# XiangLi2022/CM-TTS

Hardware: AMD Instinct MI355X
Metric: mel-frames/s (text->mel hot path, consistency sampling T=4) (higher is better)
Workload: dtype f32

## Files before the change

### cm-tts_amd/csrc/cmtts_api.hip

```cpp
#include <hip/hip_runtime.h>
#include <limits.h>
#include <math.h>
#include <stdio.h>
#include <stdlib.h>
#include <string.h>

#include <algorithm>
#include <map>
#include <string>
#include <vector>

#include "../../include/cmtts_hip.h"
#include "internal_hooks.h"
#include "conv_args.h"
#include "kernels.h"
#include "resblock_args.h"
#include "persist_args.h"
#include "cond_gemm.h"
#include "resblock_pair.h"
#include "inproj.h"
#include "attention.h"
#include "text_state.h"
#include "stream_windows.h"

// ... 385 lines not shown
int launch(const ConvArgs& a, int epi, int nbatch, hipStream_t s) {
    const int r = cmtts_launch_conv(&a, epi, nbatch, (void*)s);
    if (r != 0) return fail(r, "conv launch failed (unsupported shape or HIP launch error)");
    return 0;
}

struct Carver {
    char* base;
    size_t off = 0;
    explicit Carver(void* b) : base((char*)b) {}
    template <class T>
    T* take(size_t n) {
        off = (off + 255) & ~(size_t)255;
        T* p = (T*)(base + off);
        off += n * sizeof(T);
        return p;
    }
};

struct Profile {
    bool on = false;
    std::vector<hipEvent_t> ev;
    size_t used = 0;
    int stride = 1;
    long seen = 0;
} g_prof;

bool g_fused_resblock = true;
int g_persist_tail = 1;
extern "C" int cmtts_launch_conv_xresq(const ConvArgs* a, const float* wq, int nbatch, void* stream, int form);
int g_ffn_wino = 1;
int g_ffn_fused = 1;
int g_inproj_fused = 1;
int g_step_cache = 1;
int g_persist_wino = 3;
int g_voc_wino = 1;
int g_voc_wino64_k = 7;
int g_voc_wino43 = 1;
int g_voc_qpair = 1;
int g_voc_wino64 = 1;
int g_voc_pair3 = 1;
int g_voc_pairw = 1;
int g_voc_pair128 = 1;
int g_voc_rb16 = 1;
int g_voc_upsT = 1;
int g_voc_xl16 = 1;
int g_pred_xl = 1;
int g_pred_head = 1;
int g_text_xres = 7;
int g_attn_fused = 1;
int g_voc_xl = 1;
int g_voc_pair = 1;
int g_qkv_nt = 0;
int g_stats_mlp = 1;
int g_cwt_in_phoneme = 1;
int g_xres_small = 1;
int g_ffn_xres = 1;
int g_split_resblock = 1;
int g_cond_gemm16 = 1;
int g_cond_gemm = 1;
int g_persist = 1;
unsigned* g_tmo_host = nullptr;
int check_device_flag(bool before_launch = false) {
    if (!g_tmo_host) return 0;
    unsigned v = __atomic_load_n(g_tmo_host, __ATOMIC_RELAXED);
    if (!v) return 0;
// ... 784 lines not shown
int g_cond_inkernel = 1;
inline bool C_IS_256(const cmtts_config& c) { return c.res_channels == 256; }
bool CondFactors::usable(const cmtts_model* m) const {
    return g_cond_factored && p1 && mel2ph && p_idx && m->precision == 0 && m->cond_p2 && g_fused_resblock;
}
int cond_factored(cmtts_model* m, const DenWs& w, const CondFactors& f, int B, int T, hipStream_t s) {
    const cmtts_config& c = m->cfg;
    const int r = cmtts_launch_cond_expand(f.p1, f.ldp, f.L, m->cond_p2, c.pitch_bins, f.mel2ph, f.p_idx, w.cp, B, c.res_layers * c.res_channels, T, (void*)s);
    return r == 0 ? 0 : fail(CMTTS_E_HIP, "cond_expand launch failed");
}
int cond_phoneme_factor(cmtts_model* m, const float* out1, int B, int Lp, float* p1, hipStream_t s) {
    const cmtts_config& c = m->cfg;
    if (!m->cond_p2) return fail(CMTTS_E_UNSUPPORTED, "factored conditioner projections are not available for this model");
    CondGemmArgs g;
    memset(&g, 0, sizeof(g));
    g.X = out1; g.Wf = m->cond_all_f; g.bias = m->cond_zero_bias; g.Y = p1;
    g.B = B; g.T = Lp; g.M = c.res_layers * c.res_channels; g.K = c.hidden; g.force = 1;
    g.flat = 1;
    const long tiles = ((long)B * Lp + 63) / 64;
    const int npass = g.M / 512;
    int best = 1;
    double best_t = 1e30;
    for (int sp = 1; sp <= npass; ++sp) {
        const int ppg = (npass + sp - 1) / sp, groups = (npass + ppg - 1) / ppg;
        const long wg = tiles * groups, cap = persist_blocks();
        const double t = (double)((wg + cap - 1) / cap) * ppg;
        if (t < best_t - 1e-9) { best_t = t; best = sp; }
    }
    g.row_split = best;
    const int r = cmtts_launch_cond_gemm(&g, (void*)s);
    return r == 0 ? 0 : fail(r == -2 ? CMTTS_E_UNSUPPORTED : CMTTS_E_HIP, "cond_gemm (phoneme factor) launch failed");
}

int step_embedding(cmtts_model* m, const DenWs& w, const float* timesteps, const float* spk, int B, hipStream_t s,
                   float t_host = NAN) {
    const cmtts_config& c = m->cfg;
    const int C = c.res_channels, NL = c.res_layers;
    if (c.multi_speaker && !spk) return fail(CMTTS_E_INVALID, "speaker_emb is required for a multi-speaker model");
    const bool cacheable = g_step_cache && t_host == t_host;
    if (cacheable) {
        for (const cmtts_model::StepRow& e : m->step_rows)
            if (e.t == t_host && hipEventQuery(e.ready) == hipSuccess) {
                k_broadcast_row(e.row, w.dproj, B, NL * C, s);
                if (c.multi_speaker) {
                    k_dense_small(spk, c.hidden, 1, m->sproj_wt, nullptr, nullptr, w.sproj, B, c.hidden, NL * C, DENSE_NONE, s);
                    k_add_rows(w.dproj, w.sproj, w.dp, (long)B * NL * C, s);
                }
                return 0;
            }
    }
    k_diff_embed(timesteps, m->omega_res, w.emb, B, C, s);
    k_dense_small(w.emb, C, 1, m->mlp0_wt, nullptr, nullptr, w.e1, B, C, 4 * C, DENSE_MISH, s);
    k_dense_small(w.e1, 4 * C, 1, m->mlp2_wt, nullptr, nullptr, w.e2, B, 4 * C, C, DENSE_NONE, s);
    k_dense_small(w.e2, C, 1, m->dproj_wt, nullptr, nullptr, w.dproj, B, C, NL * C, DENSE_NONE, s);
    if (c.multi_speaker) {
        k_dense_small(spk, c.hidden, 1, m->sproj_wt, nullptr, nullptr, w.sproj, B, c.hidden, NL * C, DENSE_NONE, s);
        k_dense_small(w.e2, C, 1, m->dproj_wt, nullptr, w.sproj, w.dp, B, C, NL * C, DENSE_NONE, s);
    }
    if (cacheable && m->step_rows.size() < 16) {
        bool known = false;
        for (const cmtts_model::StepRow& e : m->step_rows) known = known || e.t == t_host;
        if (!known) {
            cmtts_model::StepRow e{t_host, nullptr, nullptr};
            void* p = nullptr;
            if (hipMalloc(&p, (size_t)NL * C * sizeof(float)) == hipSuccess && hipEventCreateWithFlags(&e.ready, hipEventDisableTiming) == hipSuccess) {
                e.row = (float*)p;
// ... 24 lines not shown
    *halo_zeroed = false;
    int rin = -2;
    if (g_inproj_fused && m->in_proj_f) {
        InProjArgs ia;
        memset(&ia, 0, sizeof(ia));
        ia.x = x_src; ia.scale = in_scale; ia.wf = m->in_proj_f; ia.bias = m->in_proj.bias; ia.h = w.h;
        ia.B = B; ia.T = T; ia.M = M; ia.C = C;
        const bool persist_path = g_fused_resblock && g_persist && NL <= PERSIST_MAX_LAYERS;
        if (persist_path) { ia.zero = w.halo; ia.zero_f4 = (long)(cmtts_persist_halo_bytes(B, T) / 16); }
        rin = cmtts_launch_inproj(&ia, (void*)s);
        if (rin == -3) return fail(CMTTS_E_HIP, "inproj launch failed");
        *halo_zeroed = rin == 0 && persist_path && cmtts_persist_halo_bytes(B, T) % 16 == 0;
    }
    if (rin != 0) {
        k_mel_prep(x_src, nullptr, in_scale, w.hin, B, T, M, s);
        ConvArgs a = conv_args(m->in_proj, w.hin, T, T, (long)M * T, w.h, T, cs, T);
        a.out[0].act = ACT_RELU;
        CHK(launch(a, EPI_PLAIN, B, s));
    }
    if (embed) CHK(step_embedding(m, w, timesteps, spk, B, s, t_host));
    return 0;
}

int batch_invariant_form(const cmtts_model* m) {
    if (!m->batch_invariant || m->precision != 0 || !m->winograd || !g_persist_wino || !m->res[0].w3w) return 0;
    return m->winograd == 1 && g_persist_wino == 3 && m->res[0].w3w43 ? 1 : -1;
}
int check_batch_invariant(const cmtts_model* m) {
    if (batch_invariant_form(m) >= 0) return 0;
    return fail(CMTTS_E_UNSUPPORTED, "batch_invariant: the persistent denoiser stack runs the F(2,3) form (model option \"winograd\" = 2), "
                                     "which has no per-layer counterpart; set \"winograd\" to 1 or 0");
}

int denoiser_core(cmtts_model* m, const DenWs& w, const float* x_src, float in_scale, const float* timesteps,
                  const float* cond_ct, const float* spk, int B, int T, const MelPost& post, hipStream_t s, bool embed = true,
                  SideStream* pending = nullptr, float t_host = NAN,
                  const CondFactors* cfk = nullptr, bool* cp_ready = nullptr) {
    CHK(check_device_flag(true));
    const cmtts_config& c = m->cfg;
    const int C = c.res_channels, NL = c.res_layers, M = c.n_mels;
    const long cs = (long)C * T;
    bool halo_zeroed = false;
    CHK(denoiser_prologue(m, w, x_src, in_scale, timesteps, spk, B, T, s, embed, t_host, &halo_zeroed));
    if (pending) CHK(branch_join(pending));
    const float* dp = m->cfg.multi_speaker ? w.dp : w.dproj;
    const bool unfused = !g_fused_resblock;
    float* hcur = w.h;
    float* halt = w.u;
    bool layers_done = false;
    if (!unfused && g_persist && NL <= PERSIST_MAX_LAYERS) {
        PersistArgs pa;
        memset(&pa, 0, sizeof(pa));
        pa.x0 = w.h; pa.cp = w.cp; pa.cp_bstride = (long)NL * C * T;
        pa.dp = dp; pa.d = w.dproj; pa.vec_stride = (long)NL * C;
        pa.skip = w.skip; pa.halo = w.halo; pa.tmo = g_tmo_host;
        pa.B = B; pa.T = T; pa.NL = NL;
        pa.halo_zeroed = halo_zeroed;
        const int prec = m->precision;
        if (cfk && !(cp_ready && *cp_ready)) {
            pa.fact = 1; pa.p1 = cfk->p1; pa.p2 = m->cond_p2; pa.mel2ph = (const long long*)cfk->mel2ph; pa.pidx = (const long long*)cfk->p_idx;
            pa.ldp = cfk->ldp; pa.Lph = cfk->L; pa.ld2 = c.pitch_bins;
            pa.p1t = cfk->p1t; pa.p2t = m->cond_p2t;
        }
        if (g_persist_tail && m->skip_f && m->outp_f) {
            pa.tail = 1;
            pa.Wsf = m->skip_f; pa.bs = m->skip_proj.bias; pa.Wpf = m->outp_f; pa.bp = m->out_proj.bias;
            pa.skip_div = (float)sqrt((double)NL); pa.n_mels = M;
            pa.xold = post.xold; pa.noise = post.noise; pa.c_out = post.c_out; pa.c_skip = post.c_skip; pa.nstd = post.nstd;
            pa.out = post.out;
        }
        pa.wino = g_persist_wino && m->winograd && !prec && m->res[0].w3w && w.pst;
        if (pa.wino && g_persist_wino == 3 && m->winograd == 1 && m->res[0].w3w43) pa.wino = 3;
        pa.xst = w.pst;
        for (int l = 0; l < NL; ++l) {
            pa.W3f[l] = prec ? (const float*)m->res[l].w3f16[prec - 1] : (pa.wino == 3 ? m->res[l].w3w43 : pa.wino ? m->res[l].w3w : m->res[l].w3f);
            pa.Wof[l] = prec ? (const float*)m->res[l].wof16[prec - 1] : m->res[l].wof;
            pa.b3[l] = m->res[l].b3f; pa.bo[l] = m->res[l].outp.bias;
        }
        const bool prof = g_prof.on && g_prof.used + 2 <= g_prof.ev.size();
        const int need = cmtts_persist_plan(B, T, NL, persist_blocks(), g_persist == 2);
        if (need) CHK(persist_admit(s, need, persist_blocks()));
        if (prof) (void)hipEventRecord(g_prof.ev[g_prof.used], s);
        const int rc = prec ? cmtts_launch_denoiser_persist_lp(&pa, prec, persist_blocks(), g_persist == 2, (void*)s)
                            : cmtts_launch_denoiser_persist(&pa, persist_blocks(), g_persist == 2, (void*)s);
        if (rc == -3) return fail(CMTTS_E_HIP, "persistent denoiser launch failed");
        if (rc == 0) {
            CHK(persist_launched(s, need));
            if (prof) { (void)hipEventRecord(g_prof.ev[g_prof.used + 1], s); g_prof.used += 2; }
            layers_done = true;
            if (pa.tail) return 0;
        }
    }
    if (!layers_done && cfk && !(cp_ready && *cp_ready)) {
        CHK(cond_factored(m, w, *cfk, B, T, s));
        if (cp_ready) *cp_ready = true;
    }
    const bool w43 = batch_invariant_form(m) > 0;
    for (int l = 0; l < NL && !layers_done; ++l) {
        const ResLayer& R = m->res[l];
        const bool prof = g_prof.on && g_prof.used + 2 <= g_prof.ev.size() && (g_prof.seen++ % g_prof.stride) == 0;
        if (!unfused) {
            ResArgs ra;
            memset(&ra, 0, sizeof(ra));
            ra.x_in = hcur; ra.cp = w.cp + (long)l * C * T; ra.cp_bstride = (long)NL * C * T;
            ra.dp = dp + (long)l * C; ra.d = w.dproj + (long)l * C;
            ra.x_out = halt; ra.skip = w.skip;
            ra.W3f = R.w3f; ra.b3 = R.b3f; ra.Wof = R.wof; ra.bo = R.outp.bias;
            ra.vec_stride = (long)NL * C; ra.B = B; ra.T = T; ra.accum_skip = l > 0; ra.flag = g_tmo_host;
            if (prof) (void)hipEventRecord(g_prof.ev[g_prof.used], s);
            int lrc;
            if (m->precision == 0 || m->precision == 3) {
                const long tiles32 = (long)((T + 31) / 32) * B;
                ra.z = w.zb;
                if (w43) {
                    ra.W3f = R.w3w43;
                    lrc = cmtts_launch_resblock_w43(&ra, (void*)s);
                } else if (g_split_resblock == 2 || (g_split_resblock == 1 && tiles32 <= SPLIT_MAX_TILES)) lrc = cmtts_launch_resblock_split(&ra, (void*)s);
                else lrc = cmtts_launch_resblock(&ra, (void*)s);
// ... 547 lines not shown
    if (g_fused_resblock) CHK(cond_projections(m, w, cond_ct, B, T, ss ? ss->side : s));
    const MelPost post = {nullptr, nullptr, 1.0f, 0.0f, 0.0f, out};
    CHK(denoiser_core(m, w, x, 1.0f, timesteps, cond_ct, speaker_emb, B, T, post, s, true, ss));
    HIPCHK(hipGetLastError());
    return 0;
}

int cmtts_schedule(const cmtts_model* m, int n_steps, float* sigmas, float* renoise_std) {
    if (!m || !sigmas || !renoise_std || n_steps < 1) return fail(CMTTS_E_INVALID, "cmtts_schedule: bad argument");
    const cmtts_config& c = m->cfg;
    if (n_steps == 1) {
        sigmas[0] = c.sigma_max;
        renoise_std[0] = -1.0f;
        return 0;
    }
    const double rho = c.rho, tmax = pow((double)c.sigma_max, 1.0 / rho), tmin = pow((double)c.sigma_min, 1.0 / rho);
    for (int i = 0; i < n_steps; ++i) {
        const double tsi = 0.0, tsn = (i + 1 == n_steps) ? 1.0 : 0.0;
        const double t = pow(tmax + tsi / 1.0 * (tmin - tmax), rho);
        double nt = pow(tmax + tsn / 1.0 * (tmin - tmax), rho);
        nt = nt < c.sigma_min ? (double)c.sigma_min : (nt > c.sigma_max ? (double)c.sigma_max : nt);
        sigmas[i] = (float)t;
        renoise_std[i] = (float)sqrt(nt * nt - (double)c.sigma_min * (double)c.sigma_min);
    }
    return 0;
}

}
namespace {
int sample_core(cmtts_model* m, const DenWs& w, const float* noise, long noise_stride, const float* cond_ct, const float* speaker_emb, int B,
                int T, int n_steps, const float* sigmas, const float* renoise_std, float* mel, hipStream_t s, const CondFactors* cf = nullptr) {
    const cmtts_config& c = m->cfg;
    const long nel = (long)B * T * c.n_mels;
    SideStream* ss = g_fused_resblock ? side_for(s) : nullptr;
    if (ss) CHK(branch_fork(ss));
    const CondFactors* cfk = nullptr;
    CondFactors cf_local;
    bool cp_ready = false;
    if (g_fused_resblock) {
        if (cf && cf->usable(m)) {
            const bool inkernel = g_cond_inkernel && g_persist && g_persist_tail && m->skip_f && m->outp_f && c.res_layers <= PERSIST_MAX_LAYERS &&
                                  cmtts_persist_plan(B, T, c.res_layers, persist_blocks(), g_persist == 2) > 0;
            if (inkernel && cf->ldp <= T && m->cond_p2t && C_IS_256(c)) {
                cf_local = *cf;
                if (!cf_local.p1t) {
                    k_transpose(cf->p1, w.cp, B * c.res_layers, c.res_channels, cf->ldp, ss ? ss->side : s);
                    cf_local.p1t = w.cp;
                }
                cfk = &cf_local;
            } else CHK(cond_factored(m, w, *cf, B, T, ss ? ss->side : s));
        } else CHK(cond_projections(m, w, cond_ct, B, T, ss ? ss->side : s));
    }
    k_scale(noise, w.xcur, nel, c.sigma_max, s);
    const float smin = c.sigma_min, sd2 = c.sigma_data * c.sigma_data;
    for (int i = 0; i < n_steps; ++i) {
        const float sg = sigmas[i];
        const float dm = sg - smin;
        const float c_skip = sd2 / (dm * dm + sd2);
        const float rt = sqrtf(sg * sg + sd2);
        const float c_out = dm * c.sigma_data / rt;
        const float c_in = 1.0f / rt;
        const float t_resc = 250.0f * logf(sg + 1e-44f);
        const bool new_sigma = i == 0 || sigmas[i] != sigmas[i - 1];
        const bool embed_side = i == 0 && ss != nullptr;
        if (new_sigma) k_fill_float(w.tbuf, t_resc, B, embed_side ? ss->side : s);
        if (embed_side) CHK(step_embedding(m, w, w.tbuf, speaker_emb, B, ss->side, t_resc));
        const bool last = i + 1 == n_steps;
        const bool renoise = renoise_std[i] >= 0.0f;
        const MelPost post = {w.xcur, renoise ? noise + (long)(1 + i) * noise_stride : nullptr, c_out, c_skip,
                              renoise ? renoise_std[i] : 0.0f, last ? mel : w.xcur};
        CHK(denoiser_core(m, w, w.xcur, c_in, w.tbuf, cond_ct, speaker_emb, B, T, post, s, new_sigma && !embed_side, i == 0 ? ss : nullptr, t_resc, cfk, &cp_ready));
    }
    HIPCHK(hipGetLastError());
    return 0;
}

DenWs den_slice(const cmtts_config& c, const DenWs& w, int b0, int T) {
    const long C = c.res_channels, NL = c.res_layers, M = c.n_mels;
    DenWs v = w;
    v.hin += (long)b0 * M * T; v.h += b0 * C * T; v.u += b0 * C * T; v.zb += b0 * C * T; v.skip += b0 * C * T;
    v.emb += b0 * C; v.e1 += b0 * 4 * C; v.e2 += b0 * C; v.dproj += b0 * NL * C; v.sproj += b0 * NL * C; v.dp += b0 * NL * C;
    v.tbuf += b0; v.xcur += (long)b0 * T * M; v.cp += (long)b0 * NL * C * T;
    return v;
}
}
extern "C" {

int cmtts_sample(cmtts_model* m, const float* noise, const float* cond_ct, const float* speaker_emb, int B, int T,
                 int n_steps, const float* sigmas, const float* renoise_std, float* mel, void* ws, size_t ws_bytes,
                 void* stream) {
    if (!m || !m->finalized) return fail(CMTTS_E_INVALID, "model not finalized");
    if (!noise || !cond_ct || !mel || !ws || !sigmas || !renoise_std || B <= 0 || T <= 0 || n_steps < 1)
        return fail(CMTTS_E_INVALID, "cmtts_sample: bad argument");
    CHK(check_batch_invariant(m));
    const cmtts_config& c = m->cfg;
    DenWs w = carve_den(c, B, T, ws);
    if (ws_bytes < w.bytes) return fail(CMTTS_E_WORKSPACE, "denoiser workspace too small");
    return sample_core(m, w, noise, (long)B * T * c.n_mels, cond_ct, speaker_emb, B, T, n_steps, sigmas, renoise_std, mel, (hipStream_t)stream);
}

int cmtts_sample_factored(cmtts_model* m, const float* noise, const float* cond_ct, const float* speaker_emb, int B, int T,
                          int n_steps, const float* sigmas, const float* renoise_std, float* mel, void* ws, size_t ws_bytes,
                          void* stream, const float* cond_p1, int p1_ld, int L, const int64_t* mel2ph, const int64_t* p_idx) {
    return cmtts_sample_factored_t(m, noise, cond_ct, speaker_emb, B, T, n_steps, sigmas, renoise_std, mel, ws, ws_bytes, stream, cond_p1, nullptr, p1_ld, L,
// ... 687 lines not shown
    bool found;
    const int prev = knob_set(tab, sizeof(tab) / sizeof(tab[0]), name, value, &found);
    if (found) return prev;
    return fail(CMTTS_E_INVALID, "cmtts_model_set_option: unknown option");
}

int cmtts_vocoder_set_option(cmtts_vocoder* v, const char* name, int value) {
    if (!v || !name) return fail(CMTTS_E_INVALID, "cmtts_vocoder_set_option: null argument");
    const Knob tab[] = {
        {"ups16", &v->ups16, 0, 1},
        {"winograd", &v->winograd, 0, 1},
        {"batch_invariant", &v->batch_invariant, 0, 1},
    };
    bool found;
    const int prev = knob_set(tab, sizeof(tab) / sizeof(tab[0]), name, value, &found);
    if (found) return prev;
    return fail(CMTTS_E_INVALID, "cmtts_vocoder_set_option: unknown option");
}

int cmtts_internal_set(const char* name, int value) {
    if (!name) return fail(CMTTS_E_INVALID, "cmtts_internal_set: null name");
    static const Knob tab[] = {
        {"qkv_nt", &g_qkv_nt, 0, 3},
        {"cwt_in_phoneme", &g_cwt_in_phoneme, 0, 1},
        {"pred_xres", &g_pred_xres, 0, 1},
        {"xres_small", &g_xres_small, 0, 1},
        {"cond_inkernel", &g_cond_inkernel, 0, 1},
        {"cond_factored", &g_cond_factored, 0, 1},
        {"cond_gemm16", &g_cond_gemm16, 0, 1},
        {"cond_gemm", &g_cond_gemm, 0, 2},
        {"persist_tail", &g_persist_tail, 0, 1},
        {"persist_wino", &g_persist_wino, 0, 3},
        {"inproj_fused", &g_inproj_fused, 0, 1},
        {"ffn_xres", &g_ffn_xres, 0, 1},
        {"ffn_wino", &g_ffn_wino, 0, 2},
        {"ffn_fused", &g_ffn_fused, 0, 1},
        {"text_xres", &g_text_xres, 0, 15},
        {"attn_fused", &g_attn_fused, 0, 1},
        {"pred_xl", &g_pred_xl, 0, 1},
        {"pred_head", &g_pred_head, 0, 1},
        {"voc_pair", &g_voc_pair, 0, 2},
        {"voc_pair3", &g_voc_pair3, 0, 1},
        {"voc_pairw", &g_voc_pairw, 0, 1},
        {"voc_pair128", &g_voc_pair128, 0, 1},
        {"voc_rb16", &g_voc_rb16, 0, 2},
        {"voc_xl", &g_voc_xl, 0, 1},
        {"voc_wino64_k", &g_voc_wino64_k, 3, 99},
        {"voc_wino43", &g_voc_wino43, 0, 3},
        {"voc_qpair", &g_voc_qpair, 0, 2},
        {"voc_wino64", &g_voc_wino64, 0, 1},
        {"voc_wino", &g_voc_wino, 0, 2},
        {"voc_xl16", &g_voc_xl16, 0, 1},
        {"voc_upsT", &g_voc_upsT, 0, 1},
        {"post_v4", &g_post_v4, 0, 1},
        {"pred_wino", &g_pred_wino, 0, 1},
        {"energy_head", &g_energy_head, 0, 1},
        {"stats_mlp", &g_stats_mlp, 0, 1},
        {"text_xt16", &g_conv_xt16, 0, 1},
    };
    if (!strcmp(name, "voc_xl_split")) return cmtts_xl_set_split(value);
    if (!strcmp(name, "attn_qb")) return cmtts_attention_set_qb(value);
    if (!strcmp(name, "xres_nt")) return cmtts_xres_set_nt(value);
    bool found;
    const int prev = knob_set(tab, sizeof(tab) / sizeof(tab[0]), name, value, &found);
    if (found) return prev;
    return fail(CMTTS_E_INVALID, "cmtts_internal_set: unknown switch");
// ... 196 lines not shown
```

### cm-tts_amd/csrc/denoiser_persist.hip

```cpp
#include <hip/hip_runtime.h>
#include <type_traits>
#include "gate.h"
#include "persist_args.h"
#include "persist_tail.h"
#include "wino43.h"

typedef float f32x16 __attribute__((ext_vector_type(16)));
typedef float f32x4 __attribute__((ext_vector_type(4)));
typedef float f32x2 __attribute__((ext_vector_type(2)));
typedef __attribute__((address_space(1))) unsigned long long gu64;

#ifndef WINO_ABL
#define WINO_ABL 0
#endif
#ifndef WINO_L2PF
#define WINO_L2PF 0
#endif
#ifndef WINO_THREAD
#define WINO_THREAD 1
#endif
#ifndef WINO43_RING
#define WINO43_RING 3
#endif
#ifndef WINO_RING
// ... 50 lines not shown
    const float* dp_b = (RAGGED ? a.grp[gi].dp : a.dp) + (long)b * a.vec_stride;
    const float* dv_b = (RAGGED ? a.grp[gi].d : a.d) + (long)b * a.vec_stride;
    unsigned long long* halo_g = RAGGED ? a.grp[gi].halo : a.halo;
    const int B_g = RAGGED ? a.grp[gi].B : a.B, tiles_g = RAGGED ? a.grp[gi].tiles : a.tiles;
    const int mrow0 = w * 32;
    const float *p1_b = nullptr, *p1t_b = nullptr;
    const long long *m2p_b = nullptr, *pix_b = nullptr;
    int ldp = 0, Lph = 0;
    if (FACT) {
        p1_b = (RAGGED ? a.grp[gi].p1 : a.p1);
        ldp = RAGGED ? a.grp[gi].ldp : a.ldp;
        Lph = RAGGED ? a.grp[gi].Lph : a.Lph;
        p1_b += (long)b * a.NL * C * ldp;
        p1t_b = (RAGGED ? a.grp[gi].p1t : a.p1t) + (long)b * a.NL * C * ldp;
        m2p_b = (RAGGED ? a.grp[gi].mel2ph : a.mel2ph) + (long)b * T;
        pix_b = (RAGGED ? a.grp[gi].pidx : a.pidx) + (long)b * T;
    }
    auto frame_idx = [&](int t_c, int& ph, int& ix) {
        const long long p = m2p_b[t_c], q = pix_b[t_c];
        ph = (int)(p > Lph ? Lph : p);
        ix = q < 0 ? 0 : (q >= a.ld2 ? a.ld2 - 1 : (int)q);
    };
    auto cp_fact = [&](int row, int ph, int ix) -> float {
        const float av = p1_b[(long)row * ldp + (ph > 0 ? ph - 1 : 0)];
        const float qv = a.p2[(long)row * a.ld2 + ix];
        return (ph > 0 ? av : 0.f) + qv;
    };

    auto uidx = [](int f) { return WINO == 1 ? ((f & 1) ? (f + 1) >> 1 : 33 + (f >> 1)) : f + 1; };
    constexpr int PST_TILE = NW * 8 * 64 * 4;
    float* pst_b = nullptr;
    if (WINO) pst_b = (RAGGED ? a.grp[gi].xst : a.xst) + ((long)b * (RAGGED ? a.grp[gi].tiles : a.tiles) + tile) * PST_TILE;

    {
        const float* xin = x0_b;
        const int t = t0 + lane;
        const int t_c = min(t, T - 1);
        int ph0 = 0, ix0 = 0;
        if (FACT) frame_idx(t_c, ph0, ix0);
        constexpr int ROWS_PER_WAVE = C / NW;
#pragma unroll 1
        for (int i = 0; i < ROWS_PER_WAVE; i += 8) {
            float xv[8], cv[8], dq[8];
#pragma unroll
            for (int q = 0; q < 8; ++q) {
                const int m = w * ROWS_PER_WAVE + i + q;
                xv[q] = xin[(unsigned)(m * T + t_c)];
                cv[q] = FACT ? cp_fact(m, ph0, ix0) : cp_b[(unsigned)(m * T + t_c)];
                dq[q] = dp_b[m];
            }
#pragma unroll
            for (int q = 0; q < 8; ++q) {
                const int m = w * ROWS_PER_WAVE + i + q;
                const float uv = cv[q] + (xv[q] + dq[q]);
                smem[m * U_LD + uidx(lane)] = t < Tc ? uv : 0.f;
            }
        }
        if (tid < 2 * C) {
            const int m = tid & (C - 1);
            const bool right = tid >= C;
            const int th = right ? t0 + FN : t0 - 1;
            const int thc = min(max(th, 0), T - 1);
            float cph0;
            if (FACT) { int ph, ix; frame_idx(thc, ph, ix); cph0 = cp_fact(m, ph, ix); }
            else cph0 = cp_b[(unsigned)(m * T + thc)];
            const float uh = cph0 + (xin[(unsigned)(m * T + thc)] + dp_b[m]);
            smem[m * U_LD + uidx(right ? FN : -1)] = (th >= 0 && th < Tc) ? uh : 0.f;
        }
    }
    int* idx_lds = reinterpret_cast<int*>(smem + 2 * C * U_LD);
    int* zflag = idx_lds + (FN + 2) * 2 + NW * 64;
    if (tid < NW) zflag[tid] = 0;
    if (FACT && tid < FN + 2) {
        int ph, ix;
        frame_idx(min(max(t0 - 1 + tid, 0), T - 1), ph, ix);
        idx_lds[2 * tid] = ph;
        idx_lds[2 * tid + 1] = ix;
    }
    f32x16 st[MT][NT];
    {
        const float* xin = x0_b;
#pragma unroll
        for (int i = 0; i < MT; ++i)
#pragma unroll
            for (int j = 0; j < NT; ++j) {
                const int t_c = min(t0 + j * 32 + l31, T - 1);
#pragma unroll
                for (int r = 0; r < 16; ++r)
                    st[i][j][r] = (i == 0 && !WINO) ? ldg(xin, (unsigned)((mrow0 + acc_row(r, lane)) * T + t_c)) : 0.f;
            }
    }

    f32x16 acc[MT][NT];
    auto load_a = [&](f32x4 (&dst)[MT], const float* wfrag, int group) {
#pragma unroll
        for (int i = 0; i < MT; ++i)
            dst[i] = *reinterpret_cast<const f32x4*>(wfrag + ((long)group * (2 * C / 32) + w * MT + i) * 256 + lane * 4);
    };
    auto load_ao = [&](f32x4 (&dst)[MT], const float* wfrag, int group) {
#pragma unroll
        for (int i = 0; i < MT; ++i)
            dst[i] = *reinterpret_cast<const f32x4*>(wfrag + ((long)group * (2 * C / 32) + i * NW + w) * 256 + lane * 4);
    };
    const f32x16 zero16 = {0.f, 0.f, 0.f, 0.f, 0.f, 0.f, 0.f, 0.f, 0.f, 0.f, 0.f, 0.f, 0.f, 0.f, 0.f, 0.f};
    auto mma_group = [&](auto first, const f32x4 (&af)[MT], const float (&bv)[4][NT], auto i0) {
        constexpr bool FIRST = decltype(first)::value;
        constexpr int I0 = decltype(i0)::value;
#pragma unroll
        for (int kk = 0; kk < 4; ++kk)
#pragma unroll
            for (int i = I0; i < MT; ++i)
#pragma unroll
                for (int j = 0; j < NT; ++j)
                    acc[i][j] = __builtin_amdgcn_mfma_f32_32x32x2f32(af[i][kk], bv[kk][j], FIRST && kk == 0 ? zero16 : acc[i][j], 0, 0, 0);
    };
    using first_t = std::integral_constant<bool, true>;
    using later_t = std::integral_constant<bool, false>;

    const int bid_dbg = blockIdx.x + gridDim.x * blockIdx.y;
#ifdef PUB_STAMP
    constexpr bool PUBS = true;
#else
    constexpr bool PUBS = false;
// ... 261 lines not shown
                    bf[i][r] = ldg(b3, (unsigned)(mg + 16));
                }
            if constexpr (WINO == 1) {
#pragma unroll
                for (int i = 0; i < MT; ++i)
#pragma unroll
                    for (int r = 0; r < 8; ++r) {
                        const float ge = (accw[i][0][r] + accw[i][1][r]) + accw[i][2][r];
                        const float go = (accw[i][1][r] - accw[i][2][r]) - accw[i][3][r];
                        const float fe = (accw[i][0][r + 8] + accw[i][1][r + 8]) + accw[i][2][r + 8];
                        const float fo = (accw[i][1][r + 8] - accw[i][2][r + 8]) - accw[i][3][r + 8];
                        float2 zz;
                        zz.x = cmtts_gate(ge + bg[i][r], fe + bf[i][r]);
                        zz.y = cmtts_gate(go + bg[i][r], fo + bf[i][r]);
                        *reinterpret_cast<float2*>(z_lds + ((w * MT + i) * 16 + acc_row(r, ln)) * U_LD + 2 * (ln & 31)) = zz;
                    }
            } else {
#pragma unroll
            for (int i = 0; i < MT; ++i)
#pragma unroll
                for (int j = 0; j < NT; ++j)
#pragma unroll
                    for (int r = 0; r < 8; ++r) {
                        const float zv = cmtts_gate(acc[i][j][r] + bg[i][r], acc[i][j][r + 8] + bf[i][r]);
                        z_lds[((w * MT + i) * 16 + acc_row(r, ln)) * U_LD + j * 32 + (ln & 31)] = zv;
                    }
            }
        }
        float l2touch = 0.f;
        if constexpr (WINO) {
#pragma unroll
            for (int s = 0; s < RING - 1; ++s) load_ao(A[s], a.Wof[l], min(s, NGC - 1));
            const int ln = opaque(lane);
            if (l == 0) {
#pragma unroll
                for (int j = 0; j < NT; ++j) {
                    const int t_c = min(t0 + j * 32 + (ln & 31), T - 1);
#pragma unroll
                    for (int r = 0; r < 16; ++r) st[0][j][r] = ldg(x0_b, (unsigned)((mrow0 + acc_row(r, ln)) * T + t_c));
                }
            } else {
                const f32x4* px = reinterpret_cast<const f32x4*>(pst_b) + (w * 8) * 64 + ln;
#pragma unroll
                for (int j = 0; j < NT; ++j)
#pragma unroll
                    for (int q = 0; q < 4; ++q) {
                        const f32x4 vx = px[(j * 4 + q) * 64];
#pragma unroll
                        for (int e = 0; e < 4; ++e) st[0][j][4 * q + e] = vx[e];
                    }
            }
#if WINO_L2PF
            if (more) {
                const int bid = blockIdx.x + gridDim.x * blockIdx.y;
                const unsigned line = (unsigned)((((bid >> 3) & 31) * NW + w) * 64 + ln);
                l2touch = *reinterpret_cast<const float*>(reinterpret_cast<const char*>(a.W3f[l + 1]) + (size_t)line * 128u);
            }
#endif
        }
        stamp(l, 3);
        if (lane == 0) __hip_atomic_store(zflag + w, l + 1, __ATOMIC_RELEASE, __HIP_MEMORY_SCOPE_WORKGROUP);
        unsigned zready = 0;
        auto need_z = [&](int v) {
            if (v >= NW || ((zready >> v) & 1u)) return;
            unsigned spins = 0;
            for (;;) {
                const int f = __hip_atomic_load(zflag + (lane & (NW - 1)), __ATOMIC_ACQUIRE, __HIP_MEMORY_SCOPE_WORKGROUP);
// ... 53 lines not shown
                ring_round(0, first_t{}, std::integral_constant<int, 1>{});
#pragma unroll 1
                for (int it = RING; it < NG; it += RING) ring_round(it, later_t{}, std::integral_constant<int, 1>{});
            }
        }
        stamp(l, 5);
        {
            const float* bo = a.bo[l];
            const float* dl = dv_b + (long)l * C;
            const int ln = opaque(lane);
            float bor[MT][16], ddr[16];
#pragma unroll
            for (int r = 0; r < 16; ++r) {
                bor[0][r] = ldg(bo, (unsigned)(mrow0 + acc_row(r, ln)));
                bor[1][r] = ldg(bo, (unsigned)(C + mrow0 + acc_row(r, ln)));
                ddr[r] = ldg(dl, (unsigned)(mrow0 + acc_row(r, ln)));
            }
            if (WINO) asm volatile("" ::"v"(l2touch));
#pragma unroll
            for (int j = 0; j < NT; ++j)
#pragma unroll
                for (int r = 0; r < 16; ++r) {
                    const float o = acc[0][j][r] + bor[0][r];
                    st[0][j][r] = (o + (st[0][j][r] + ddr[r])) * CMTTS_RSQRT2;
                    const float os = acc[1][j][r] + bor[1][r];
                    st[1][j][r] = l > 0 ? os + st[1][j][r] : os;
                }
        }
        if (!more) break;
        stamp(l, 6);
        pstamp(l, 0);
        __builtin_amdgcn_sched_barrier(0);
        const float* dpn = dp_b + (long)(l + 1) * C;
        const unsigned tag = (unsigned)l + 1;
        unsigned long long* hbase = halo_g + ((((long)(l & 1) * B_g + b) * tiles_g) * 2) * C;
        {
            const int ln = opaque(lane), c31 = ln & 31;
            float* edge = reinterpret_cast<float*>(smem + 2 * C * U_LD) + (FN + 2) * 2 + w * 64;
            if (c31 == 0) {
#pragma unroll
                for (int r = 0; r < 16; ++r) edge[acc_row(r, ln)] = st[0][0][r];
            }
            if (c31 == 31) {
#pragma unroll
                for (int r = 0; r < 16; ++r) edge[32 + acc_row(r, ln)] = st[0][NT - 1][r];
            }
            store_granule(hbase + ((long)tile * 2 + (ln >> 5)) * C + mrow0 + (ln & 31), tag, edge[ln]);
        }
        const int hside = opaque(lane) >> 5, hm = mrow0 + (opaque(lane) & 31);
        const int hth = hside ? t0 + FN : t0 - 1;
        const bool hinside = hth >= 0 && hth < Tc;
        const unsigned long long* hg = hbase + ((long)(hinside ? (hside ? tile + 1 : tile - 1) : tile) * 2 + (hside ? 0 : 1)) * C + hm;
        float hcp = 0.f;
        int hph = 0, hix = 0;
        {
            const int thc = min(max(hth, 0), T - 1);
            if (FACT) { hph = idx_lds[2 * (hside ? FN + 1 : 0)]; hix = idx_lds[2 * (hside ? FN + 1 : 0) + 1]; }
            else hcp = (cp_b + (long)(l + 1) * C * T)[(unsigned)(hm * T + thc)];
        }
        unsigned long long hv = __hip_atomic_load((gu64*)hg, __ATOMIC_RELAXED, __HIP_MEMORY_SCOPE_AGENT);
        pstamp(l, 1);
        {
            const float* cpn = cp_b + (long)(l + 1) * C * T;
            const int ln = opaque(lane), c31 = ln & 31;
            f32x16 cpc[NT];
            float dpr[16];
            if constexpr (FACT) {
// ... 158 lines not shown
extern "C" size_t cmtts_persist_halo_bytes(int B, int T) {
    const long tiles = (T + FN - 1) / FN;
    return (size_t)2 * B * tiles * 2 * C * sizeof(unsigned long long);
}

extern "C" int cmtts_launch_denoiser_persist(const PersistArgs* a_in, int max_blocks, int force, void* stream_) {
    PersistArgs a = *a_in;
    hipStream_t stream = (hipStream_t)stream_;
    const int tiles = (a.T + FN - 1) / FN;
    if (a.NL < 1 || a.NL > PERSIST_MAX_LAYERS || tiles > max_blocks || (long)C * a.T >= (1L << 30)) return -2;
    if (!force && (long)tiles * a.B * 2 <= (long)max_blocks) return -2;
    a.tiles = tiles;
    a.dbg = g_pdbg;
    if ((a.wino == 1 || a.wino == 3) && !a.xst) return -2;
    const int wsel = a.wino == 3 ? 2 : a.wino ? 1 : 0;
    if (a.wino == 2) return -2;
    const int threads = 64 * NW;
#define KFN(D, R, F, W) reinterpret_cast<const void*>(denoiser_persist_kernel<D, R, F, W>)
    static const void* const kfns[2][2][3] = {
        {{KFN(false, false, false, 0), KFN(false, false, false, 1), KFN(false, false, false, 2)}, {KFN(false, false, true, 0), KFN(false, false, true, 1), KFN(false, false, true, 2)}},
        {{KFN(true, false, false, 0), KFN(true, false, false, 1), KFN(true, false, false, 2)}, {KFN(true, false, true, 0), KFN(true, false, true, 1), KFN(true, false, true, 2)}}};
    static bool attr_set = false;
    const size_t lds = (size_t)2 * C * U_LD * sizeof(float) + IDX_LDS_BYTES;
    if (!attr_set) {
        for (int d = 0; d < 2; ++d)
            for (int f = 0; f < 2; ++f) {
                for (int wn = 0; wn < 3; ++wn)
                    if (hipFuncSetAttribute(kfns[d][f][wn], hipFuncAttributeMaxDynamicSharedMemorySize, (int)lds) != hipSuccess) return -3;
            }
        attr_set = true;
    }
    if (a.fact && (!a.p1 || !a.p2 || !a.mel2ph || !a.pidx || a.ldp < 1 || a.ld2 < 1)) return -2;
    if (a.fact && (!a.p1t || !a.p2t)) return -2;
    if (!a.halo_zeroed && hipMemsetAsync(a.halo, 0, cmtts_persist_halo_bytes(a.B, a.T), stream) != hipSuccess) return -3;
    const int B = a.B;
    const int per_launch = max_blocks / tiles;
    const int nchunks = (B + per_launch - 1) / per_launch;
    const int bc = (B + nchunks - 1) / nchunks;
    for (int b0 = 0; b0 < B; b0 += bc) {
        PersistArgs c = a;
        const int nb = B - b0 < bc ? B - b0 : bc;
        c.x0 = a.x0 + (long)b0 * C * a.T;
        c.cp = a.cp + (long)b0 * a.cp_bstride;
        c.dp = a.dp + (long)b0 * a.vec_stride;
        c.d = a.d + (long)b0 * a.vec_stride;
        c.skip = a.skip + (long)b0 * C * a.T;
        if (a.xst) c.xst = a.xst + (long)b0 * tiles * (NW * 8 * 64 * 4);
        c.halo = a.halo + (long)b0 * tiles * 2 * C;
        if (a.fact) {
            c.p1 = a.p1 + (long)b0 * a.NL * C * a.ldp;
            if (a.p1t) c.p1t = a.p1t + (long)b0 * a.NL * C * a.ldp;
            c.mel2ph = a.mel2ph + (long)b0 * a.T;
            c.pidx = a.pidx + (long)b0 * a.T;
        }
        if (a.tail) {
            const long off = (long)b0 * a.T * a.n_mels;
            c.xold = a.xold ? a.xold + off : nullptr;
            c.noise = a.noise ? a.noise + off : nullptr;
            c.out = a.out + off;
        }
        const void* kfn = kfns[a.dbg ? 1 : 0][a.fact ? 1 : 0][wsel];
        void* params[] = {(void*)&c};
        const int variant = wsel * 2 + (a.fact ? 1 : 0);
        if (!a.dbg && cmtts_persist_cooperative(variant, tiles, nb)) {
            if (hipLaunchCooperativeKernel(kfn, dim3(tiles, nb), dim3(threads), params, (unsigned)lds, stream) != hipSuccess) return -3;
            cmtts_persist_validated(variant, tiles, nb);
        } else if (hipLaunchKernel(kfn, dim3(tiles, nb), dim3(threads), params, lds, stream) != hipSuccess) return -3;
        if (hipGetLastError() != hipSuccess) return -3;
    }
    return 0;
}

extern "C" int cmtts_launch_denoiser_persist_ragged(const PersistArgs* a_in, void* stream_) {
    const PersistArgs& a = *a_in;
    hipStream_t stream = (hipStream_t)stream_;
    if (a.NL < 1 || a.NL > PERSIST_MAX_LAYERS || a.n_groups < 1 || a.n_groups > PERSIST_MAX_GROUPS || a.n_wg < 1 || a.n_wg > PERSIST_MAX_WG)
        return -2;
    for (int g = 0; g < a.n_groups; ++g)
        if ((long)C * a.grp[g].T >= (1L << 30) || a.grp[g].tiles > 127 || a.grp[g].B > 1023) return -2;
    static const void* const kfns[2][3] = {{KFN(false, true, false, 0), KFN(false, true, false, 1), KFN(false, true, false, 2)},
                                           {KFN(false, true, true, 0), KFN(false, true, true, 1), KFN(false, true, true, 2)}};
    static bool attr_set = false;
    const size_t lds = (size_t)2 * C * U_LD * sizeof(float) + IDX_LDS_BYTES;
    if (!attr_set) {
        for (int f = 0; f < 2; ++f) {
            for (int wn = 0; wn < 3; ++wn)
                if (hipFuncSetAttribute(kfns[f][wn], hipFuncAttributeMaxDynamicSharedMemorySize, (int)lds) != hipSuccess) return -3;
        }
        attr_set = true;
    }
    if (a.fact) {
        if (!a.p2 || a.ld2 < 1) return -2;
// ... 22 lines not shown
```

### cm-tts_amd/csrc/persist_args.h

```cpp
#pragma once
#include <stddef.h>

#define PERSIST_MAX_LAYERS 32
#define PERSIST_MAX_GROUPS 8
#define PERSIST_MAX_WG 256

struct PersistGroup {
    const float* x0;
    const float* cp;
    const float* dp;
    const float* d;
    float* skip;
    unsigned long long* halo;
    const float* xold;
    const float* noise;
    float* out;
    long cp_bstride;
    int B, T, tiles, pad_;
    const float* p1;
    const long long* mel2ph;
    const long long* pidx;
    int ldp, Lph;
    const float* p1t;
    float* xst;
// ... 7 lines not shown
    float* skip;
    const float* W3f[PERSIST_MAX_LAYERS];
    const float* b3[PERSIST_MAX_LAYERS];
    const float* Wof[PERSIST_MAX_LAYERS];
    const float* bo[PERSIST_MAX_LAYERS];
    unsigned long long* halo;
    unsigned* tmo;
    long cp_bstride;
    long vec_stride;
    int B, T, NL;
    int tiles;
    int tail;
    const float* Wsf;
    const float* bs;
    const float* Wpf;
    const float* bp;
    float skip_div;
    int n_mels;
    const float* xold;
    const float* noise;
    float c_out, c_skip, nstd;
    float* out;
    int fact;
    const float* p1;
    const float* p2;
    const long long* mel2ph;
    const long long* pidx;
    int ldp, Lph, ld2;
    const float* p1t;
    const float* p2t;
    int wino;
    float* xst;
    int halo_zeroed;
    long long* dbg;
    int n_groups;
    int n_wg;
    PersistGroup grp[PERSIST_MAX_GROUPS];
    unsigned desc[PERSIST_MAX_WG];
};

#ifdef __cplusplus
extern "C" {
#endif
size_t cmtts_persist_halo_bytes(int B, int T);
size_t cmtts_persist_state_floats(int B, int T);
int cmtts_launch_denoiser_persist(const PersistArgs* a, int max_blocks, int force, void* stream);
int cmtts_launch_denoiser_persist_lp(const PersistArgs* a, int mode, int max_blocks, int force, void* stream);
int cmtts_launch_denoiser_persist_ragged(const PersistArgs* a, void* stream);
int cmtts_persist_plan(int B, int T, int NL, int max_blocks, int force);
int cmtts_persist_chunks(int B, int T, int max_blocks);
void cmtts_persist_set_debug(long long* dbg);
long long* cmtts_persist_get_debug(void);
int cmtts_persist_set_cooperative(int on);
void cmtts_persist_validated(int variant, int gx, int gy);
int cmtts_persist_cooperative(int variant, int gx, int gy);
int cmtts_persist_note_process_group(int on);
#ifdef __cplusplus
}
#endif
```

### cm-tts_amd/csrc/persist_tail.h

```cpp
#pragma once
#include <hip/hip_runtime.h>
#include "persist_args.h"

namespace persist_tail {

typedef float f32x16 __attribute__((ext_vector_type(16)));
typedef float f32x4 __attribute__((ext_vector_type(4)));
constexpr int PT_C = 256, PT_NT = 2, PT_LD = 68, PT_RING = 6;

__device__ __forceinline__ int pt_opaque(int v) { asm volatile("" : "+v"(v)); return v; }
__device__ __forceinline__ float pt_ldg(const float* base, unsigned idx) {
    return *reinterpret_cast<const float*>(reinterpret_cast<const char*>(base) + (size_t)(idx * 4u));
}
__device__ __forceinline__ int pt_row(int r, int lane) { return (r & 3) + 8 * (r >> 2) + 4 * (lane >> 5); }

template <int TPW = 1>
__device__ __forceinline__ void run(const PersistArgs& a, float* u_lds, float* z_lds, const f32x16* skip, int w, int lane,
                                    int b, int t0, int T, const float* xold, const float* noise, float* out, int Tc) {
    constexpr int C = PT_C, NT = PT_NT, U_LD = PT_LD, RING = PT_RING;
    const int l31 = lane & 31, khalf = lane >> 5;
    auto opaque = [](int v) { return pt_opaque(v); };
    auto acc_row = [](int r, int ln) { return pt_row(r, ln); };
    auto ldg = [](const float* p, unsigned i) { return pt_ldg(p, i); };
    {
// ... 51 lines not shown
        const int mrow0 = (w * TPW + i) * 32;
        gemm_tile(a.Wsf, C / 32, w * TPW + i, u_lds);
        const int ln = opaque(lane), c31 = ln & 31;
#pragma unroll
        for (int r = 0; r < 16; ++r) {
            const int m = mrow0 + acc_row(r, ln);
            const float bi = ldg(a.bs, (unsigned)m);
#pragma unroll
            for (int j = 0; j < NT; ++j) {
                float v = h[j][r] + bi;
                v *= 1.0f;
                v = v > 0.f ? v : 0.f;
                z_lds[m * U_LD + j * 32 + c31] = v;
            }
        }
    }
    __syncthreads();
    const int otiles = (a.n_mels + 31) / 32;
    if (w < otiles) {
        const int mrow0 = w * 32;
        gemm_tile(a.Wpf, otiles, w, z_lds);
        const int ln = opaque(lane), c31 = ln & 31;
        const int M = a.n_mels;
        float bi[16];
#pragma unroll
        for (int r = 0; r < 16; ++r) bi[r] = ldg(a.bp, (unsigned)min(mrow0 + acc_row(r, ln), M - 1));
        bool bad = false;
#pragma unroll
        for (int j = 0; j < NT; ++j) {
            const int t = t0 + j * 32 + c31;
            const long ob = ((long)b * T + min(t, T - 1)) * M;
            float xo[16], nz[16];
            if (xold) {
#pragma unroll
                for (int r = 0; r < 16; ++r) xo[r] = xold[ob + min(mrow0 + acc_row(r, ln), M - 1)];
            }
            if (noise) {
#pragma unroll
                for (int r = 0; r < 16; ++r) nz[r] = noise[ob + min(mrow0 + acc_row(r, ln), M - 1)];
            }
#pragma unroll
            for (int r = 0; r < 16; ++r) {
                const int m = mrow0 + acc_row(r, ln);
                const bool ok = m < M && t < Tc;
                const float F = h[j][r] + (m < M ? bi[r] : 0.f);
                float v = a.c_out * F;
                if (xold) v = __builtin_fmaf(a.c_skip, xo[r], v);
                if (noise) v = __builtin_fmaf(nz[r] * a.nstd, 0.85f, v);
                if (ok) out[ob + m] = v;
                bad |= ok && !(fabsf(v) <= 3.402823466e38f);
            }
        }
        if (bad && a.tmo && *(volatile unsigned*)a.tmo == 0u) *(volatile unsigned*)a.tmo = 2u;
    }
}

}
```

Before: 1.975 million.

## Fuse denoiser input projection into persistent kernel and skip cached step embeddings

Moves the mel input projection (80->256 conv with ReLU, including halo columns) into the prologue of the persistent denoiser kernel using MFMA, so the separate prologue conv launch and the initial noise scaling kernel are no longer needed. When the step embedding row for a sigma is already cached, the kernel reads it directly with zero batch stride, and the side-stream fork is skipped when no side work remains. Halo tags are offset per step so the halo buffer is zeroed once per sampling run instead of before every step. This adds shared-memory and register pressure to the kernel head and restricts the path to n_mels=80, C=256 and fp32.

```diff
diff --git a/cm-tts_amd/csrc/cmtts_api.hip b/cm-tts_amd/csrc/cmtts_api.hip
--- a/cm-tts_amd/csrc/cmtts_api.hip
+++ b/cm-tts_amd/csrc/cmtts_api.hip
@@ -441,6 +441,7 @@
 int g_ffn_wino = 1;
 int g_ffn_fused = 1;
 int g_inproj_fused = 1;
+int g_inproj_inkernel = 1;
 int g_step_cache = 1;
 int g_persist_wino = 3;
 int g_voc_wino = 1;
@@ -1291,6 +1292,12 @@
     return r == 0 ? 0 : fail(r == -2 ? CMTTS_E_UNSUPPORTED : CMTTS_E_HIP, "cond_gemm (phoneme factor) launch failed");
 }
 
+const float* cached_step_row(const cmtts_model* m, float t_host) {
+    if (!g_step_cache || t_host != t_host) return nullptr;
+    for (const cmtts_model::StepRow& e : m->step_rows)
+        if (e.t == t_host && hipEventQuery(e.ready) == hipSuccess) return e.row;
+    return nullptr;
+}
 int step_embedding(cmtts_model* m, const DenWs& w, const float* timesteps, const float* spk, int B, hipStream_t s,
                    float t_host = NAN) {
     const cmtts_config& c = m->cfg;
@@ -1381,16 +1388,26 @@
                                      "which has no per-layer counterpart; set \"winograd\" to 1 or 0");
 }
 
+struct HeadIn {
+    float xin_scale;
+    unsigned tag0;
+    const float* step_row;
+};
+
 int denoiser_core(cmtts_model* m, const DenWs& w, const float* x_src, float in_scale, const float* timesteps,
                   const float* cond_ct, const float* spk, int B, int T, const MelPost& post, hipStream_t s, bool embed = true,
                   SideStream* pending = nullptr, float t_host = NAN,
-                  const CondFactors* cfk = nullptr, bool* cp_ready = nullptr) {
+                  const CondFactors* cfk = nullptr, bool* cp_ready = nullptr,
+                  const HeadIn* hin = nullptr) {
     CHK(check_device_flag(true));
     const cmtts_config& c = m->cfg;
     const int C = c.res_channels, NL = c.res_layers, M = c.n_mels;
     const long cs = (long)C * T;
     bool halo_zeroed = false;
-    CHK(denoiser_prologue(m, w, x_src, in_scale, timesteps, spk, B, T, s, embed, t_host, &halo_zeroed));
+    if (hin) {
+        if (embed) CHK(step_embedding(m, w, timesteps, spk, B, s, t_host));
+        halo_zeroed = true;
+    } else CHK(denoiser_prologue(m, w, x_src, in_scale, timesteps, spk, B, T, s, embed, t_host, &halo_zeroed));
     if (pending) CHK(branch_join(pending));
     const float* dp = m->cfg.multi_speaker ? w.dp : w.dproj;
     const bool unfused = !g_fused_resblock;
@@ -1405,6 +1422,11 @@
         pa.skip = w.skip; pa.halo = w.halo; pa.tmo = g_tmo_host;
         pa.B = B; pa.T = T; pa.NL = NL;
         pa.halo_zeroed = halo_zeroed;
+        if (hin) {
+            pa.inproj = 1; pa.xin = x_src; pa.xin_scale = hin->xin_scale; pa.in_scale = in_scale;
+            pa.Winf = m->in_proj_f; pa.bin = m->in_proj.bias; pa.tag0 = hin->tag0;
+            if (hin->step_row) { pa.dp = pa.d = hin->step_row; pa.vec_stride = 0; }
+        }
         const int prec = m->precision;
         if (cfk && !(cp_ready && *cp_ready)) {
             pa.fact = 1; pa.p1 = cfk->p1; pa.p2 = m->cond_p2; pa.mel2ph = (const long long*)cfk->mel2ph; pa.pidx = (const long long*)cfk->p_idx;
@@ -1433,6 +1455,7 @@
         const int rc = prec ? cmtts_launch_denoiser_persist_lp(&pa, prec, persist_blocks(), g_persist == 2, (void*)s)
                             : cmtts_launch_denoiser_persist(&pa, persist_blocks(), g_persist == 2, (void*)s);
         if (rc == -3) return fail(CMTTS_E_HIP, "persistent denoiser launch failed");
+        if (rc != 0 && hin) return fail(CMTTS_E_UNSUPPORTED, "persistent denoiser launch refused the in-kernel input projection");
         if (rc == 0) {
             CHK(persist_launched(s, need));
             if (prof) { (void)hipEventRecord(g_prof.ev[g_prof.used + 1], s); g_prof.used += 2; }
@@ -2046,16 +2069,23 @@
                 int T, int n_steps, const float* sigmas, const float* renoise_std, float* mel, hipStream_t s, const CondFactors* cf = nullptr) {
     const cmtts_config& c = m->cfg;
     const long nel = (long)B * T * c.n_mels;
-    SideStream* ss = g_fused_resblock ? side_for(s) : nullptr;
+    const bool one_launch = g_fused_resblock && g_persist && g_persist_tail && m->skip_f && m->outp_f && c.res_layers <= PERSIST_MAX_LAYERS &&
+                            cmtts_persist_plan(B, T, c.res_layers, persist_blocks(), g_persist == 2) > 0;
+    const bool head = one_launch && g_inproj_inkernel && g_inproj_fused && m->precision == 0 && m->in_proj_f && c.n_mels == 80 && C_IS_256(c) &&
+                      c.res_layers >= 2 && !((uintptr_t)noise & 15) && !((uintptr_t)w.xcur & 15);
+    const bool fact_inkernel = cf && cf->usable(m) && g_cond_inkernel && one_launch && cf->ldp <= T && m->cond_p2t && C_IS_256(c);
+    const float t_resc0 = 250.0f * logf(sigmas[0] + 1e-44f);
+    const float* row0 = head && !c.multi_speaker ? cached_step_row(m, t_resc0) : nullptr;
+    const bool side_work = !head || !row0 || !(fact_inkernel && cf->p1t);
+    SideStream* ss = g_fused_resblock && side_work ? side_for(s) : nullptr;
     if (ss) CHK(branch_fork(ss));
+    if (head) HIPCHK(hipMemsetAsync(w.halo, 0, cmtts_persist_halo_bytes(B, T), ss ? ss->side : s));
     const CondFactors* cfk = nullptr;
     CondFactors cf_local;
     bool cp_ready = false;
     if (g_fused_resblock) {
         if (cf && cf->usable(m)) {
-            const bool inkernel = g_cond_inkernel && g_persist && g_persist_tail && m->skip_f && m->outp_f && c.res_layers <= PERSIST_MAX_LAYERS &&
-                                  cmtts_persist_plan(B, T, c.res_layers, persist_blocks(), g_persist == 2) > 0;
-            if (inkernel && cf->ldp <= T && m->cond_p2t && C_IS_256(c)) {
+            if (fact_inkernel) {
                 cf_local = *cf;
                 if (!cf_local.p1t) {
                     k_transpose(cf->p1, w.cp, B * c.res_layers, c.res_channels, cf->ldp, ss ? ss->side : s);
@@ -2065,8 +2095,9 @@
             } else CHK(cond_factored(m, w, *cf, B, T, ss ? ss->side : s));
         } else CHK(cond_projections(m, w, cond_ct, B, T, ss ? ss->side : s));
     }
-    k_scale(noise, w.xcur, nel, c.sigma_max, s);
+    if (!head) k_scale(noise, w.xcur, nel, c.sigma_max, s);
     const float smin = c.sigma_min, sd2 = c.sigma_data * c.sigma_data;
+    const float* step_row = nullptr;
     for (int i = 0; i < n_steps; ++i) {
         const float sg = sigmas[i];
         const float dm = sg - smin;
@@ -2076,14 +2107,19 @@
         const float c_in = 1.0f / rt;
         const float t_resc = 250.0f * logf(sg + 1e-44f);
         const bool new_sigma = i == 0 || sigmas[i] != sigmas[i - 1];
-        const bool embed_side = i == 0 && ss != nullptr;
-        if (new_sigma) k_fill_float(w.tbuf, t_resc, B, embed_side ? ss->side : s);
+        if (new_sigma) step_row = i == 0 ? row0 : (head && !c.multi_speaker ? cached_step_row(m, t_resc) : nullptr);
+        const bool embed_now = new_sigma && !step_row;
+        const bool embed_side = embed_now && i == 0 && ss != nullptr;
+        if (embed_now) k_fill_float(w.tbuf, t_resc, B, embed_side ? ss->side : s);
         if (embed_side) CHK(step_embedding(m, w, w.tbuf, speaker_emb, B, ss->side, t_resc));
         const bool last = i + 1 == n_steps;
         const bool renoise = renoise_std[i] >= 0.0f;
-        const MelPost post = {w.xcur, renoise ? noise + (long)(1 + i) * noise_stride : nullptr, c_out, c_skip,
+        const float* xsrc = head && i == 0 ? noise : w.xcur;
+        const MelPost post = {xsrc, renoise ? noise + (long)(1 + i) * noise_stride : nullptr, c_out, c_skip,
                               renoise ? renoise_std[i] : 0.0f, last ? mel : w.xcur};
-        CHK(denoiser_core(m, w, w.xcur, c_in, w.tbuf, cond_ct, speaker_emb, B, T, post, s, new_sigma && !embed_side, i == 0 ? ss : nullptr, t_resc, cfk, &cp_ready));
+        const HeadIn hin = {i == 0 ? c.sigma_max : 1.0f, (unsigned)i * (unsigned)c.res_layers, step_row};
+        CHK(denoiser_core(m, w, xsrc, c_in, w.tbuf, cond_ct, speaker_emb, B, T, post, s, embed_now && !embed_side, i == 0 ? ss : nullptr, t_resc, cfk, &cp_ready,
+                          head ? &hin : nullptr));
     }
     HIPCHK(hipGetLastError());
     return 0;
@@ -2837,6 +2873,7 @@
         {"persist_tail", &g_persist_tail, 0, 1},
         {"persist_wino", &g_persist_wino, 0, 3},
         {"inproj_fused", &g_inproj_fused, 0, 1},
+        {"inproj_inkernel", &g_inproj_inkernel, 0, 1},
         {"ffn_xres", &g_ffn_xres, 0, 1},
         {"ffn_wino", &g_ffn_wino, 0, 2},
         {"ffn_fused", &g_ffn_fused, 0, 1},
diff --git a/cm-tts_amd/csrc/denoiser_persist.hip b/cm-tts_amd/csrc/denoiser_persist.hip
--- a/cm-tts_amd/csrc/denoiser_persist.hip
+++ b/cm-tts_amd/csrc/denoiser_persist.hip
@@ -106,7 +106,120 @@
     float* pst_b = nullptr;
     if (WINO) pst_b = (RAGGED ? a.grp[gi].xst : a.xst) + ((long)b * (RAGGED ? a.grp[gi].tiles : a.tiles) + tile) * PST_TILE;
 
-    {
+    f32x16 st[MT][NT];
+    const bool head = !RAGGED && a.inproj;
+    if (head) {
+        constexpr int XM = 80, X_LD = FN + 3, KG = XM / 8, NF4 = (FN + 2) * (XM / 4);
+        float* xs = smem + C * U_LD;
+        f32x4 Ai[KG];
+#pragma unroll
+        for (int g = 0; g < KG; ++g) Ai[g] = *reinterpret_cast<const f32x4*>(a.Winf + (((long)g * (C / 32) + w) * 64 + lane) * 4);
+        {
+            const long e0 = ((long)b * T + t0 - 1) * XM;
+            f32x4 v[3];
+#pragma unroll
+            for (int j = 0; j < 3; ++j) {
+                const int e4 = tid + 64 * NW * j;
+                const int t = t0 - 1 + e4 / (XM / 4);
+                v[j] = (e4 < NF4 && t >= 0 && t < Tc) ? *reinterpret_cast<const f32x4*>(a.xin + e0 + 4 * e4) : (f32x4){0.f, 0.f, 0.f, 0.f};
+            }
+#pragma unroll
+            for (int j = 0; j < 3; ++j) {
+                const int e4 = tid + 64 * NW * j;
+                const int row = e4 / (XM / 4), k = 4 * (e4 - row * (XM / 4));
+                if (e4 < NF4) {
+#pragma unroll
+                    for (int i = 0; i < 4; ++i) xs[(k + i) * X_LD + row] = a.in_scale * (a.xin_scale * v[j][i]);
+                }
+            }
+        }
+        __syncthreads();
+        f32x16 hx;
+#pragma unroll
+        for (int r = 0; r < 16; ++r) { st[0][0][r] = 0.f; st[0][1][r] = 0.f; hx[r] = 0.f; }
+        {
+            const float* bl = xs + khalf * X_LD;
+            const int c0 = 1 + l31, ch = l31 == 1 ? FN + 1 : 0;
+#pragma unroll
+            for (int g = 0; g < KG; ++g)
+#pragma unroll
+                for (int kk = 0; kk < 4; ++kk) {
+                    const float* br = bl + (8 * g + 2 * kk) * X_LD;
+                    const float b0 = br[c0], b1 = br[c0 + 32], bh = br[ch];
+                    st[0][0] = __builtin_amdgcn_mfma_f32_32x32x2f32(Ai[g][kk], b0, st[0][0], 0, 0, 0);
+                    st[0][1] = __builtin_amdgcn_mfma_f32_32x32x2f32(Ai[g][kk], b1, st[0][1], 0, 0, 0);
+                    hx = __builtin_amdgcn_mfma_f32_32x32x2f32(Ai[g][kk], bh, hx, 0, 0, 0);
+                }
+        }
+        const int ln = opaque(lane), c31 = ln & 31;
+        {
+            float bi[16];
+#pragma unroll
+            for (int r = 0; r < 16; ++r) bi[r] = ldg(a.bin, (unsigned)(mrow0 + acc_row(r, ln)));
+#pragma unroll
+            for (int r = 0; r < 16; ++r) {
+#pragma unroll
+                for (int j = 0; j < NT; ++j) {
+                    const float v = st[0][j][r] + bi[r];
+                    st[0][j][r] = v > 0.f ? v : 0.f;
+                }
+                const float vh = hx[r] + bi[r];
+                hx[r] = vh > 0.f ? vh : 0.f;
+            }
+        }
+        float* edge = smem + 2 * C * U_LD + (FN + 2) * 2 + w * 64;
+        if (c31 == 0) {
+#pragma unroll
+            for (int r = 0; r < 16; ++r) edge[acc_row(r, ln)] = hx[r];
+        }
+        if (c31 == 1) {
+#pragma unroll
+            for (int r = 0; r < 16; ++r) edge[32 + acc_row(r, ln)] = hx[r];
+        }
+        const float xh = edge[ln];
+        if (WINO) {
+            f32x4* px = reinterpret_cast<f32x4*>(pst_b) + (w * 8) * 64 + ln;
+#pragma unroll
+            for (int j = 0; j < NT; ++j)
+#pragma unroll
+                for (int q = 0; q < 4; ++q) {
+                    f32x4 vx;
+#pragma unroll
+                    for (int e = 0; e < 4; ++e) vx[e] = st[0][j][4 * q + e];
+                    px[(j * 4 + q) * 64] = vx;
+                }
+        }
+#pragma unroll
+        for (int j = 0; j < NT; ++j) {
+            const int t = t0 + j * 32 + c31;
+            const int t_c = min(t, T - 1);
+            int ph0 = 0, ix0 = 0;
+            if (FACT) frame_idx(t_c, ph0, ix0);
+            float cv[16], dq[16];
+#pragma unroll
+            for (int r = 0; r < 16; ++r) {
+                const int m = mrow0 + acc_row(r, ln);
+                cv[r] = FACT ? cp_fact(m, ph0, ix0) : ldg(cp_b, (unsigned)(m * T + t_c));
+                dq[r] = ldg(dp_b, (unsigned)m);
+            }
+#pragma unroll
+            for (int r = 0; r < 16; ++r) {
+                const int m = mrow0 + acc_row(r, ln);
+                const float uv = cv[r] + (st[0][j][r] + dq[r]);
+                smem[m * U_LD + uidx(j * 32 + c31)] = t < Tc ? uv : 0.f;
+            }
+        }
+        {
+            const int hside = ln >> 5, hm = mrow0 + c31;
+            const int th = hside ? t0 + FN : t0 - 1;
+            const int thc = min(max(th, 0), T - 1);
+            float cph0;
+            if (FACT) { int ph, ix; frame_idx(thc, ph, ix); cph0 = cp_fact(hm, ph, ix); }
+            else cph0 = cp_b[(unsigned)(hm * T + thc)];
+            const float uh = cph0 + (xh + dp_b[hm]);
+            smem[hm * U_LD + uidx(hside ? FN : -1)] = (th >= 0 && th < Tc) ? uh : 0.f;
+        }
+    } else {
         const float* xin = x0_b;
         const int t = t0 + lane;
         const int t_c = min(t, T - 1);
@@ -151,18 +264,18 @@
         idx_lds[2 * tid] = ph;
         idx_lds[2 * tid + 1] = ix;
     }
-    f32x16 st[MT][NT];
     {
         const float* xin = x0_b;
 #pragma unroll
-        for (int i = 0; i < MT; ++i)
-#pragma unroll
-            for (int j = 0; j < NT; ++j) {
-                const int t_c = min(t0 + j * 32 + l31, T - 1);
-#pragma unroll
-                for (int r = 0; r < 16; ++r)
-                    st[i][j][r] = (i == 0 && !WINO) ? ldg(xin, (unsigned)((mrow0 + acc_row(r, lane)) * T + t_c)) : 0.f;
-            }
+        for (int j = 0; j < NT; ++j) {
+            const int t_c = min(t0 + j * 32 + l31, T - 1);
+#pragma unroll
+            for (int r = 0; r < 16; ++r) {
+                if (WINO) st[0][j][r] = 0.f;
+                else if (!head) st[0][j][r] = ldg(xin, (unsigned)((mrow0 + acc_row(r, lane)) * T + t_c));
+                st[1][j][r] = 0.f;
+            }
+        }
     }
 
     f32x16 acc[MT][NT];
@@ -490,7 +603,7 @@
 #pragma unroll
             for (int s = 0; s < RING - 1; ++s) load_ao(A[s], a.Wof[l], min(s, NGC - 1));
             const int ln = opaque(lane);
-            if (l == 0) {
+            if (l == 0 && !head) {
 #pragma unroll
                 for (int j = 0; j < NT; ++j) {
                     const int t_c = min(t0 + j * 32 + (ln & 31), T - 1);
@@ -610,7 +723,7 @@
         pstamp(l, 0);
         __builtin_amdgcn_sched_barrier(0);
         const float* dpn = dp_b + (long)(l + 1) * C;
-        const unsigned tag = (unsigned)l + 1;
+        const unsigned tag = a.tag0 + (unsigned)l + 1;
         unsigned long long* hbase = halo_g + ((((long)(l & 1) * B_g + b) * tiles_g) * 2) * C;
         {
             const int ln = opaque(lane), c31 = ln & 31;
@@ -835,6 +948,7 @@
     }
     if (a.fact && (!a.p1 || !a.p2 || !a.mel2ph || !a.pidx || a.ldp < 1 || a.ld2 < 1)) return -2;
     if (a.fact && (!a.p1t || !a.p2t)) return -2;
+    if (a.inproj && (!a.tail || a.n_mels != 80 || a.NL < 2 || !a.xin || !a.Winf || !a.bin || ((uintptr_t)a.xin & 15))) return -2;
     if (!a.halo_zeroed && hipMemsetAsync(a.halo, 0, cmtts_persist_halo_bytes(a.B, a.T), stream) != hipSuccess) return -3;
     const int B = a.B;
     const int per_launch = max_blocks / tiles;
@@ -861,6 +975,7 @@
             c.xold = a.xold ? a.xold + off : nullptr;
             c.noise = a.noise ? a.noise + off : nullptr;
             c.out = a.out + off;
+            if (a.inproj) c.xin = a.xin + off;
         }
         const void* kfn = kfns[a.dbg ? 1 : 0][a.fact ? 1 : 0][wsel];
         void* params[] = {(void*)&c};
diff --git a/cm-tts_amd/csrc/persist_args.h b/cm-tts_amd/csrc/persist_args.h
--- a/cm-tts_amd/csrc/persist_args.h
+++ b/cm-tts_amd/csrc/persist_args.h
@@ -63,6 +63,13 @@
     int wino;
     float* xst;
     int halo_zeroed;
+    int inproj;
+    const float* xin;
+    float xin_scale;
+    float in_scale;
+    const float* Winf;
+    const float* bin;
+    unsigned tag0;
     long long* dbg;
     int n_groups;
     int n_wg;
diff --git a/cm-tts_amd/csrc/persist_tail.h b/cm-tts_amd/csrc/persist_tail.h
--- a/cm-tts_amd/csrc/persist_tail.h
+++ b/cm-tts_amd/csrc/persist_tail.h
@@ -107,8 +107,9 @@
             const long ob = ((long)b * T + min(t, T - 1)) * M;
             float xo[16], nz[16];
             if (xold) {
+                const float xsc = a.inproj ? a.xin_scale : 1.0f;
 #pragma unroll
-                for (int r = 0; r < 16; ++r) xo[r] = xold[ob + min(mrow0 + acc_row(r, ln), M - 1)];
+                for (int r = 0; r < 16; ++r) xo[r] = xsc * xold[ob + min(mrow0 + acc_row(r, ln), M - 1)];
             }
             if (noise) {
 #pragma unroll
```

Result: no change. 1.983 million (median of 6 runs) (+0.4%).
